# xXCoffeeColaXc/WeatherConverter

Measured on AMD Instinct MI355X. Metric: 256x256 images/sec (T=1000 DDPM sample), higher is better.
Workload: dtype fp32-class (f16x3: 2-piece fp16 split MFMA, fp32 accumulate); 1 GPU; DDPM reverse sampling, UNet config.yaml @ 256px, 16 images/GPU, T=1000, 126 timed steps from t=999; global_batch=16, image_size=256, parallelism=single GPU, devices=1, hip_graph=True, stream_groups=2, x_finite=True

## Files before the change

weatherconverter_amd/csrc/wc_wino.hip:

```cpp
#include <stdlib.h>

#include "wc_x6.hpp"

#ifndef WC_ABL
#define WC_ABL 0
#endif
#ifndef WC_WINO_SCALAR
#define WC_WINO_SCALAR 0
#endif

namespace {

using namespace wcx6;

constexpr int NT = 256;

WC_DEVICE void wino_lds16(__amdgpu_buffer_rsrc_t srd, void* dst, unsigned voff, int soff) {
    __builtin_amdgcn_raw_ptr_buffer_load_lds(srd, (__attribute__((address_space(3))) void*)dst, 16, voff, soff, 0, 0);
}

struct WDev {
    const float* src0;
    int C0, ldc0;
    const float* scale;
    const float* shift;
    const float* src1;
    int C1, ldc1;
    int B, H, W, N;
    const void* w;
    const float* bias;
    const float* temb;
    int temb_ld;
    const float* res;
    int ldres;
    float* out;
    int ldo;
    int nck0, nck1;
    int a_exp;
    const float* abound;
    const float* wsinv;
    float* absmax;
    float* gn_part;
    int gn_ncb, gn_sw, gn_c0, gn_np64;
    int tiles_x, tiles_y, ntiles_n;
    const unsigned char* vpre;
    long vimg;
    const float* gb_x;
    int gb_ldx, gb_silu;
    const float* gb_sc0;
    const float* gb_sh0;
    const float* gb_gamma;
    const float* gb_beta;
    float* gb_part;
    float* gb_part3;
};

WC_DEVICE float wino_silu_grad(float y) {
    const float s = 1.0f / (1.0f + __expf(-y));
    return s * (1.0f + y * (1.0f - s));
}

constexpr int VPL = WC_SINGLE16 ? 8 : 16;

template <int TH, int BN, int MB = 2, int NW = 4, bool VP = false>
struct WTile {
    static constexpr int NT = 64 * NW;
    static constexpr int WAVES_N = BN / 32;
    static constexpr int WAVES_M = NW / WAVES_N;
    static_assert(WAVES_N * WAVES_M == NW && WAVES_M * 4 * MB == TH, "each wave owns 4 MB rows x 8 tiles x 32 channels");
    static constexpr int PBN = BN > 128 ? 128 : BN;
    static constexpr int HR = TH + 2;
    static constexpr int PSTR = HR * 128 + (VP ? 0 : 16);
    static constexpr int DPIECES = VPL * HR * 8 / 64;
    static_assert(!VP || VPL * HR * 8 == DPIECES * 64, "VP: the halo stage is a whole number of 1-KiB pieces");
    static constexpr int DPW = (DPIECES + NW - 1) / NW;
    static constexpr int HSTAGE = 16 * PSTR;
    static constexpr int CPSTR = TH * 128 + 16;
    static constexpr int CSTAGE = 8 * CPSTR;
    static constexpr int ITEMS = HR * 16;
    static constexpr int I_PER_T = (ITEMS + NT - 1) / NT;
    static constexpr int C_PER_T = TH * 16 * 4 / NT;
    static constexpr int BSTEP = PBN * 64;
    static constexpr int STEPS = 12;
};

WC_DEVICE int wg_grp(int r) { return ((r >= 4 && r < 12) || (r >= 16 && r < 20) || r >= 28) ? 1 : 0; }
WC_DEVICE int wg_idx(int r) { return r < 4 ? r : r < 12 ? r - 4 : r < 20 ? r - 8 : r < 28 ? r - 12 : r - 16; }
WC_DEVICE int wg_row(int r) { return 2 * wg_grp(r) + (wg_idx(r) >> 3); }
WC_DEVICE int wg_tile(int r) { return wg_idx(r) & 7; }

template <int TH, int BN, int PRO, bool RES, int MB = 2, int NW = 4>
__global__ __launch_bounds__(64 * NW) __attribute__((amdgpu_waves_per_eu(MB == 4 ? 1 : 2, MB == 4 ? 1 : 2)))
void conv3x3_wino_kernel(WDev p) {
    static_assert((PRO == 2 || PRO == 0 || PRO == 3) && !(PRO == 0 && RES),
                  "GN+SiLU (+ residual), pre-split GN+SiLU (+ residual) or one raw segment");
    constexpr bool VP = PRO == 3;
    using T = WTile<TH, BN, MB, NW, VP>;
    constexpr int NT = T::NT;
    extern __shared__ __attribute__((aligned(16))) unsigned char smem[];
    unsigned char* const cbase = smem + 2 * T::HSTAGE;

    const int tid = threadIdx.x;
    const int lane = tid & 63;
    const int wave = tid >> 6;
    const int wm = wave / T::WAVES_N;
    const int wn = wave % T::WAVES_N;

    const int nblk = gridDim.x;
    int bid = blockIdx.x;
    {
        int q = nblk / 8, r = nblk % 8, xcd = bid % 8;
        bid = (xcd < r ? xcd * (q + 1) : r * (q + 1) + (xcd - r) * q) + bid / 8;
    }
    const int tile_n = bid % p.ntiles_n;
    int tt = bid / p.ntiles_n;
    const int txi = tt % p.tiles_x;
    tt /= p.tiles_x;
    const int tyi = tt % p.tiles_y;
    const int b = tt / p.tiles_y;
    const int y0 = tyi * TH, x0 = txi * 16, n0 = tile_n * BN;

    int s_exp = p.a_exp;
    if ((RES || PRO == 0) && p.abound) {
        const float bnd = p.abound[b];
        const int e = (int)((__float_as_uint(bnd) >> 23) & 0xffu) - 127;
        if (bnd > 0.f) s_exp = min(s_exp, (PRO == 0 ? 12 : 13) - e);
        s_exp = max(s_exp, -100);
    }
    const float ascale = ldexpf(1.0f, s_exp), ainv = ldexpf(1.0f, -s_exp);
    const int S0 = T::STEPS * p.nck0;
    const int S = S0 + (RES ? p.nck1 : 0);
    constexpr bool RI = RES && (T::C_PER_T <= 2 || MB == 4);
    const int nri = RI ? min(p.nck0, p.nck1) : 0;
    const int ntail = RES ? p.nck1 - nri : 0;
    constexpr int WPT = T::PBN / 32;
    const unsigned wtile = (unsigned)(tile_n * (BN / T::PBN) + wn / WPT) * (unsigned)(S * T::BSTEP);

    const __amdgpu_buffer_rsrc_t srd0 = make_srd(p.src0);
    const __amdgpu_buffer_rsrc_t srd1 = make_srd(RES ? p.src1 : p.src0);
    const __amdgpu_buffer_rsrc_t srdw = make_srd(p.w);
    const __amdgpu_buffer_rsrc_t srdsc = make_srd(PRO == 2 ? p.scale : p.src0);
    const __amdgpu_buffer_rsrc_t srdsh = make_srd(PRO == 2 ? p.shift : p.src0);
    const __amdgpu_buffer_rsrc_t srdv = make_srd(VP ? (const void*)(p.vpre + (long)b * p.vimg) : (const void*)p.src0);
    unsigned voff[VP ? T::DPW : 1];
    if constexpr (VP) {
#pragma unroll
        for (int i = 0; i < T::DPW; ++i) {
            const int f = (wave + NW * i) * 64 + lane;
            const int P = f / (T::HR * 8), r = (f >> 3) % T::HR, tl = f & 7;
            const int y = y0 - 1 + r;
            voff[i] = (unsigned)y < (unsigned)p.H ? (unsigned)(((P * p.H + y) * (p.W / 2) + (x0 >> 1) + tl) * 16) : OOB;
        }
    }
    const int vchunk = VPL * p.H * (p.W / 2) * 16;
    auto dma_halo = [&](int c, int hs) {
        if constexpr (VP) {
            unsigned char* dst = smem + hs * T::HSTAGE + wave * 1024;
#pragma unroll
            for (int i = 0; i < T::DPW; ++i)
                if (T::DPIECES % NW == 0 || wave + NW * i < T::DPIECES)
                    wino_lds16(srdv, dst + i * NW * 1024, voff[i], c * vchunk);
        }
    };

    const int q = tid & 3;
    int hbase[T::I_PER_T];
    unsigned hin[T::I_PER_T];
    int hwr[T::I_PER_T];
    const int hpx = p.ldc0 * 4;
#pragma unroll
    for (int j = 0; j < T::I_PER_T; ++j) {
        const int i = tid + NT * j;
        const int hrow = i >> 4, tp = (i >> 2) & 3;
        const bool valid = i < T::ITEMS;
        const int iy = y0 - 1 + hrow;
        hin[j] = 0;
#pragma unroll
        for (int k = 0; k < 6; ++k) {
            const int ix = x0 - 1 + 4 * tp + k;
            const bool inb = valid && (unsigned)iy < (unsigned)p.H && (unsigned)ix < (unsigned)p.W;
            hin[j] |= (inb ? 1u : 0u) << k;
        }
        hbase[j] = (((b * p.H + iy) * p.W + x0 - 1 + 4 * tp) * p.ldc0 + 4 * q) * 4;
        hwr[j] = valid ? (q >> 1) * T::PSTR + (hrow * 8 + 2 * tp) * 16 + (q & 1) * 8 : -1;
    }
    f32x4 rh[T::I_PER_T][6];
    f32x4 rsc, rsh;
    auto load_ss = [&](int c) {
        if constexpr (PRO == 2) {
            const unsigned o = (unsigned)(b * p.C0 + c * 16 + 4 * q) * 4u;
            rsc = bload_f4(srdsc, o);
            rsh = bload_f4(srdsh, o);
        }
    };
    auto load_slot = [&](int j, int c) {
#pragma unroll
        for (int k = 0; k < 6; ++k)
            rh[j][k] = bload_f4s(srd0, ((hin[j] >> k) & 1u) ? (unsigned)(hbase[j] + k * hpx) : OOB, c * 64);
    };
    auto load_halo = [&](int c) {
        if constexpr (VP) return;
#pragma unroll
        for (int j = 0; j < T::I_PER_T; ++j) load_slot(j, c);
        load_ss(c);
    };
#if WC_WINO_SCALAR
    const float cu = -1.4426950408889634f * ainv;
    auto prologue = [&](int j, int k0, int k1) {
        if constexpr (PRO == 2) {
            if (j == 0 && k0 == 0) {
                rsc = rsc * ascale;
                rsh = rsh * ascale;
            }
        }
        auto act = [&](f32x4 a) {
#pragma unroll
            for (int e = 0; e < 4; ++e) {
                float v;
                if constexpr (PRO == 2) {
                    const float ap = __builtin_fmaf(a[e], rsc[e], rsh[e]);
                    const float r = __builtin_amdgcn_rcpf(1.0f + __builtin_amdgcn_exp2f(ap * cu));
                    v = ap * r;
                } else {
                    v = a[e] * ascale;
                }
                a[e] = v;
            }
            return a;
        };
#pragma unroll
        for (int k = k0; k < k1; ++k) {
            const f32x4 zero = {0.f, 0.f, 0.f, 0.f};
#if WC_WINO_SCALAR == 2
            rh[j][k] = ((hin[j] >> k) & 1u) ? act(rh[j][k]) : zero;
#else
            const f32x4 a = act(rh[j][k]);
            rh[j][k] = ((hin[j] >> k) & 1u) ? a : zero;
#endif
        }
    };
#else
    auto prologue = [&](int j, int k0, int k1) {
#pragma unroll
        for (int k = k0; k < k1; ++k) {
            f32x4 a = rh[j][k];
            if constexpr (PRO == 2 && !(WC_ABL & 2)) {
                a = a * rsc + rsh;
                if constexpr (!(WC_ABL & 1)) {
                    a.x = silu_fast(a.x); a.y = silu_fast(a.y);
                    a.z = silu_fast(a.z); a.w = silu_fast(a.w);
                }
            }
            rh[j][k] = ((hin[j] >> k) & 1u) ? a * ascale : f32x4{0.f, 0.f, 0.f, 0.f};
        }
    };
#endif
    auto transform = [&](int j, int t, int hs, int p0 = 0, int p1 = 4) {
        if (hwr[j] < 0) return;
        unsigned char* base = smem + hs * T::HSTAGE + hwr[j] + t * 16;
        const f32x4 d0 = rh[j][2 * t], d1 = rh[j][2 * t + 1], d2 = rh[j][2 * t + 2], d3 = rh[j][2 * t + 3];
#if WC_WINO_SCALAR
        f32x4 V[4];
#pragma unroll
        for (int e = 0; e < 4; ++e) {
            V[0][e] = d0[e] - d2[e];
            V[1][e] = d1[e] + d2[e];
            V[2][e] = d2[e] - d1[e];
            V[3][e] = d1[e] - d3[e];
        }
#else
        const f32x4 V[4] = {d0 - d2, d1 + d2, d2 - d1, d1 - d3};
#endif
#pragma unroll
        for (int pos = p0; pos < p1; ++pos) {
            u32x2 a0, a1;
            split2_f16(V[pos], a0, a1);
            unsigned char* d = base + pos * 2 * T::PSTR;
            *reinterpret_cast<u32x2*>(d) = a0;
            *reinterpret_cast<u32x2*>(d + 8 * T::PSTR) = a1;
        }
    };
    auto write_items = [&](int hs) {
        if constexpr (VP) return;
#pragma unroll
        for (int j = 0; j < T::I_PER_T; ++j) {
            prologue(j, 0, 6);
            transform(j, 0, hs);
            transform(j, 1, hs);
        }
    };

    f32x4 rc[2][RES ? T::C_PER_T : 1];
    const int cpx = (tid >> 2) & 15, crow0 = tid >> 6;
    const unsigned coff0 = (unsigned)(((b * p.H + y0 + crow0) * p.W + x0 + cpx) * p.ldc1 + 4 * q);
    const unsigned cstep = (unsigned)(NW * p.W * p.ldc1);
    const int cwr0 = (cpx & 1) * 2 * T::CPSTR + (q >> 1) * T::CPSTR + (crow0 * 8 + (cpx >> 1)) * 16 + (q & 1) * 8;
    auto load_centre = [&](auto P, int c, bool live = true) {
        constexpr int PV = decltype(P)::value;
        const unsigned v = live ? coff0 * 4u : OOB;
#pragma unroll
        for (int j = 0; j < T::C_PER_T; ++j)
            rc[PV][j] = bload_f4s(srd1, v, (int)(((unsigned)j * cstep + (unsigned)c * 16u) * 4u));
    };
    auto write_centre = [&](auto P, int cs) {
        constexpr int PV = decltype(P)::value;
        unsigned char* base = cbase + cs * T::CSTAGE + cwr0;
        const float sg = (cpx & 1) ? -ascale : ascale;
#pragma unroll
        for (int j = 0; j < T::C_PER_T; ++j) {
            u32x2 a0, a1;
            split2_f16(rc[PV][j] * sg, a0, a1);
            unsigned char* d = base + j * NW * 8 * 16;
            *reinterpret_cast<u32x2*>(d) = a0;
            *reinterpret_cast<u32x2*>(d + 4 * T::CPSTR) = a1;
        }
    };

    const int l32 = lane & 31;
    const int half = lane >> 5;
    int abase[MB];
#pragma unroll
    for (int mb = 0; mb < MB; ++mb) abase[mb] = ((4 * MB * wm + 4 * mb + wg_row(l32)) * 8 + wg_tile(l32)) * 16;
    const unsigned wlane = (unsigned)(half * T::PBN * 16 + ((wn % WPT) * 32 + l32) * 16);

    u32x4 wreg[3][2];
    auto load_w = [&](int set, int st) {
        int s = st < S0 ? st : S0 + nri + (st - S0);
        s = s < S ? s : S - 1;
        const int off = (int)(wtile + (unsigned)s * T::BSTEP);
#pragma unroll
        for (int pc = 0; pc < 2; ++pc) wreg[set][pc] = bload_u4s(srdw, wlane + (unsigned)(pc * 2 * T::PBN * 16), off);
    };
    u32x4 wres[2];
    auto load_wres = [&](int r) {
        const int s = S0 + r < S ? S0 + r : S - 1;
        const int off = (int)(wtile + (unsigned)s * T::BSTEP);
#pragma unroll
        for (int pc = 0; pc < 2; ++pc) wres[pc] = bload_u4s(srdw, wlane + (unsigned)(pc * 2 * T::PBN * 16), off);
    };

    f32x16 acc[4][MB];
#pragma unroll
    for (int i = 0; i < 4; ++i)
#pragma unroll
        for (int j = 0; j < MB; ++j)
#pragma unroll
            for (int r = 0; r < 16; ++r) acc[i][j][r] = 0.f;

    u32x4 fa[2][MB][2];
    auto read_a = [&](int fs, int hs, int dy, int pos) {
        const unsigned char* ha = smem + hs * T::HSTAGE + (pos * 2 + half) * T::PSTR + dy * 128;
#pragma unroll
        for (int mb = 0; mb < MB; ++mb)
#pragma unroll
            for (int pc = 0; pc < 2; ++pc)
                fa[fs][mb][pc] = *reinterpret_cast<const u32x4*>(ha + pc * 8 * T::PSTR + abase[mb]);
    };
    auto mfma_a = [&](int fs, int set, int pos) {
#pragma unroll
        for (int mb = 0; mb < MB; ++mb) acc[pos][mb] = mfma_f16(fa[fs][mb][0], wreg[set][0], acc[pos][mb]);
#pragma unroll
        for (int mb = 0; mb < MB; ++mb) {
            acc[pos][mb] = mfma_f16c(fa[fs][mb][0], wreg[set][1], acc[pos][mb]);
            acc[pos][mb] = mfma_f16c(fa[fs][mb][1], wreg[set][0], acc[pos][mb]);
        }
    };
    auto compute_res = [&](const u32x4 (&w)[2], int cs) {
        const unsigned char* ca = cbase + cs * T::CSTAGE + half * T::CPSTR;
#pragma unroll
        for (int r = 0; r < 2; ++r) {
            u32x4 fr[MB][2];
#pragma unroll
            for (int mb = 0; mb < MB; ++mb)
#pragma unroll
                for (int pc = 0; pc < 2; ++pc)
                    fr[mb][pc] = *reinterpret_cast<const u32x4*>(ca + (pc * 4 + r * 2) * T::CPSTR + abase[mb]);
#pragma unroll
            for (int mb = 0; mb < MB; ++mb) {
                f32x16& a = acc[r ? 3 : 0][mb];
                a = mfma_f16(fr[mb][0], w[0], a);
                a = mfma_f16c(fr[mb][0], w[1], a);
                a = mfma_f16c(fr[mb][1], w[0], a);
            }
        }
    };

    const std::integral_constant<int, 0> I0;
    const std::integral_constant<int, 1> I1;
    const int pv0 = (p.nck0 - 1) & 1;
    load_halo(0);
    dma_halo(0, pv0);
    if constexpr (RI) load_centre(I0, 0, nri > 0);
    load_w(0, 0);
    load_w(1, 1);
    write_items(pv0);
    if constexpr (RI) write_centre(I0, pv0);
    if constexpr (VP) asm volatile("s_waitcnt vmcnt(0)" ::: "memory");
    __syncthreads();
    constexpr int HALO_AT = T::I_PER_T == 1 ? 2 : 3;
    auto load_at = [](int j) { return T::I_PER_T == 1 ? 2 : (j == 0 ? 3 : 7); };
    auto pro_at = [](int j) { return j == 0 ? 5 : 9; };
    auto slot_work = [&](int j, int k, int hs) {
        if constexpr (VP) return;
        if constexpr (WC_ABL & 4) {
            if (k >= 0 && k < 3) prologue(j, 2 * k, 2 * k + 2);
            return;
        }
        if constexpr (T::I_PER_T == 1) {
            if (k >= 0 && k < 3) prologue(j, 2 * k, 2 * k + 2);
            if (k >= 3 && k < 7) transform(j, (k - 3) >> 1, hs, ((k - 3) & 1) * 2, ((k - 3) & 1) * 2 + 2);
        } else {
            if (k == 0) prologue(j, 0, 6);
            if (k == 1 || k == 2) transform(j, k - 1, hs);
        }
    };
    auto chunk = [&](auto P, auto L, int c) {
        constexpr int PV = decltype(P)::value;
        constexpr bool LAST = decltype(L)::value != 0;
        read_a(0, PV, 0, 0);
#pragma unroll
        for (int st = 0; st < T::STEPS; ++st) {
            if (!(WC_ABL & 8) || c == 0) load_w((st + 2) % 3, T::STEPS * c + st + 2);
            if constexpr (!LAST) {
#pragma unroll
                for (int j = 0; j < T::I_PER_T; ++j)
                    if (!(WC_ABL & 32) && st == load_at(j)) load_slot(j, c + 1);
                if (st == HALO_AT) {
                    dma_halo(c + 1, PV ^ 1);
                    load_ss(c + 1);
                    if constexpr (RI) load_centre(I0, c + 1, c + 1 < nri);
                }
            } else if constexpr (RES) {
                if (st == HALO_AT) load_centre(I0, nri, ntail > 0);
                if (st == HALO_AT + 1) load_centre(I1, nri + 1, ntail > 1);
            }
            if constexpr (RI) {
                if (st == 9) load_wres(c);
            }
            __builtin_amdgcn_sched_barrier(0);
            if (st + 1 < T::STEPS && (!(WC_ABL & 64) || c == 0)) read_a((st + 1) & 1, PV, (st + 1) >> 2, (st + 1) & 3);
            mfma_a(st & 1, st % 3, st & 3);
            if constexpr (!LAST) {
#pragma unroll
                for (int j = 0; j < T::I_PER_T; ++j) slot_work(j, st - pro_at(j), PV ^ 1);
                if constexpr (RI) {
                    if (st == 9) write_centre(I0, PV ^ 1);
                }
            }
        }
        if constexpr (RES) {
            if constexpr (RI) {
                if (c < nri) compute_res(wres, PV);
            }
            if constexpr (LAST) {
                if (ntail > 0) write_centre(I0, 1);
            }
        }
        if constexpr (VP && !LAST) asm volatile("s_waitcnt vmcnt(4)" ::: "memory");
        if constexpr (!(WC_ABL & 16)) __syncthreads();
    };
    const std::integral_constant<int, 0> NL;
    const std::integral_constant<int, 1> LL;
    {
        int c = 0;
        if (pv0) chunk(I1, NL, c++);
        for (; c + 1 < p.nck0 - 1; c += 2) {
            chunk(I0, NL, c);
            chunk(I1, NL, c + 1);
        }
        chunk(I0, LL, p.nck0 - 1);
    }
    if constexpr (RES) {
        auto tstep = [&](auto P, int k) {
            constexpr int PV = decltype(P)::value;
            compute_res(wreg[PV], PV ^ 1);
            load_w(PV, S0 + k + 2);
            load_centre(P, nri + k + 2, k + 2 < ntail);
            __builtin_amdgcn_sched_barrier(0);
            if (k + 1 < ntail) write_centre(std::integral_constant<int, PV ^ 1>{}, PV);
            __syncthreads();
        };
        int k = 0;
        for (; k + 1 < ntail; k += 2) {
            tstep(I0, k);
            tstep(I1, k + 1);
        }
        if (k < ntail) tstep(I0, k);
    }

    const long img_px = (long)b * p.H * p.W;
    const __amdgpu_buffer_rsrc_t srd_out = make_srd(p.out + img_px * p.ldo);
    const __amdgpu_buffer_rsrc_t srd_res = make_srd(p.res ? p.res + img_px * p.ldres : p.out);
    const int n = n0 + wn * 32 + l32;
    const bool nok = n < p.N;
    float eadd = (nok && p.bias) ? p.bias[n] : 0.f;
    if (nok && p.temb) eadd += p.temb[b * p.temb_ld + n];
    const float emul = nok ? p.wsinv[n] * ainv : 0.f;
    float vmax = 0.f;
    float gs1 = 0.f, gs2 = 0.f, gs3 = 0.f;
    const int so_px = 4 * p.ldo;
    const int so_rs = 4 * p.ldres;
#pragma unroll
    for (int mb = 0; mb < MB; ++mb) {
        unsigned vo[4], vr[4];
#pragma unroll
        for (int j = 0; j < 4; ++j) {
            const int row = 8 * j + 4 * half;
            const int pix = (y0 + 4 * MB * wm + 4 * mb + wg_row(row)) * p.W + x0 + 2 * wg_tile(row);
            vo[j] = (unsigned)(pix * p.ldo + n) * 4u;
            vr[j] = (unsigned)(pix * p.ldres + (nok ? n : 0)) * 4u;
        }
        float rv[2][16];
        if (p.res) {
#pragma unroll
            for (int r = 0; r < 16; ++r) {
                rv[0][r] = bload_f1s(srd_res, vr[r >> 2], (r & 3) * 2 * so_rs);
                rv[1][r] = bload_f1s(srd_res, vr[r >> 2], ((r & 3) * 2 + 1) * so_rs);
            }
        }
#pragma unroll
        for (int r = 0; r < 16; ++r) {
            const float m0 = acc[0][mb][r], m1 = acc[1][mb][r], m2 = acc[2][mb][r], m3 = acc[3][mb][r];
            float ya = ((m0 + m1) + m2) * emul + eadd;
            float yb = ((m1 - m2) - m3) * emul + eadd;
            if (p.res) {
                ya += rv[0][r];
                yb += rv[1][r];
            }
            acc[0][mb][r] = ya;
            acc[1][mb][r] = yb;
            vmax = fmaxf(vmax, fmaxf(fabsf(ya), fabsf(yb)));
        }
        if constexpr (PRO == 0) {
            if (p.gb_part) {
                const __amdgpu_buffer_rsrc_t srd_x = make_srd(p.gb_x + img_px * p.gb_ldx);
                const int so_x = 4 * p.gb_ldx;
                float xv[2][16];
#pragma unroll
                for (int r = 0; r < 16; ++r) {
                    const int j = r >> 2;
                    const int row = 8 * j + 4 * half;
                    const int pix = (y0 + 4 * MB * wm + 4 * mb + wg_row(row)) * p.W + x0 + 2 * wg_tile(row);
                    const unsigned vx = nok ? (unsigned)(pix * p.gb_ldx + n) * 4u : OOB;
                    xv[0][r] = bload_f1s(srd_x, vx, (r & 3) * 2 * so_x);
                    xv[1][r] = bload_f1s(srd_x, vx, ((r & 3) * 2 + 1) * so_x);
                }
                const long bn = (long)b * p.N + (nok ? n : 0);
                const float sc0 = p.gb_sc0[bn], sh0 = p.gb_sh0[bn];
                const float ga = p.gb_gamma ? p.gb_gamma[nok ? n : 0] : 1.f;
                const float be = p.gb_beta ? p.gb_beta[nok ? n : 0] : 0.f;
#pragma unroll
                for (int r = 0; r < 16; ++r)
#pragma unroll
                    for (int e = 0; e < 2; ++e) {
                        const float xh = xv[e][r] * sc0 + sh0;
                        float d = acc[e][mb][r];
                        if (p.gb_silu) d *= wino_silu_grad(ga * xh + be);
                        gs1 += d;
                        gs2 += d * xh;
                        gs3 += xh;
                    }
            }
        }
        if (nok) {
            if constexpr (WC_ABL & 128) {
                float sum = 0.f;
#pragma unroll
                for (int r = 0; r < 16; ++r) sum += acc[0][mb][r] + acc[1][mb][r];
                if (sum == 1234.5678f) bstore_f1s(srd_out, vo[0], 0, sum);
            } else {
#pragma unroll
                for (int r = 0; r < 16; ++r) {
                    bstore_f1s(srd_out, vo[r >> 2], (r & 3) * 2 * so_px, acc[0][mb][r]);
                    bstore_f1s(srd_out, vo[r >> 2], ((r & 3) * 2 + 1) * so_px, acc[1][mb][r]);
                }
            }
        }
    }
    if (!nok) vmax = 0.f;
    if (p.absmax) block_absmax_atomic(p.absmax, b, vmax);
    if constexpr (PRO == 0) {
        if (p.gb_part) {
            gs1 += __shfl_xor(gs1, 32, 64);
            gs2 += __shfl_xor(gs2, 32, 64);
            gs3 += __shfl_xor(gs3, 32, 64);
            const int splits = p.tiles_y * p.tiles_x * T::WAVES_M;
            const long sp = (long)b * splits + ((long)tyi * p.tiles_x + txi) * T::WAVES_M + wm;
            if (nok && half == 0) {
                p.gb_part[(sp * p.N + n) * 2] = gs1;
                p.gb_part[(sp * p.N + n) * 2 + 1] = gs2;
                if (p.gb_part3) p.gb_part3[sp * p.N + n] = gs3;
            }
        }
    }
    if (p.gn_part) {
        const int r4 = tyi * (TH / 4) + MB * wm;
#pragma unroll
        for (int mb = 0; mb < MB; ++mb) {
            const f32x16 blk[2][1] = {{acc[0][mb]}, {acc[1][mb]}};
            GnTile g{p.gn_part, p.gn_ncb, p.gn_sw,
                     (long)b * p.gn_np64 + (long)(((r4 + mb) >> 1) * p.tiles_x + txi) * 2 + ((r4 + mb) & 1),
                     (p.gn_c0 + n0 + wn * 32) / 32};
            gn_tile_partials(blk, g, p.N - n0 - wn * 32 >= 32 ? 1 : 0);
        }
    }
}

template <int TH, int BN, int PRO, bool RES, int MB = 2, int NW = 4>
int launch_wino(const WDev& d, hipStream_t stream) {
    using T = WTile<TH, BN, MB, NW, PRO == 3>;
    constexpr int lds = 2 * T::HSTAGE + (RES ? 2 * T::CSTAGE : 0);
    static bool attr_set = false;
    if (!attr_set) {
        hipError_t e = hipFuncSetAttribute(reinterpret_cast<const void*>(&conv3x3_wino_kernel<TH, BN, PRO, RES, MB, NW>),
                                           hipFuncAttributeMaxDynamicSharedMemorySize, lds);
        if (e != hipSuccess) return (int)e;
        attr_set = true;
    }
    WDev p = d;
    p.tiles_x = p.W / 16;
    p.tiles_y = p.H / TH;
    p.ntiles_n = (p.N + BN - 1) / BN;
    dim3 grid(p.B * p.tiles_y * p.tiles_x * p.ntiles_n);
    WC_SET_NAME("conv3x3_wino_kernel", {WC_TI(TH), WC_TI(BN), WC_TI(PRO), WC_TB(RES), WC_TI(MB), WC_TI(NW)});
    hipLaunchKernelGGL((conv3x3_wino_kernel<TH, BN, PRO, RES, MB, NW>), grid, dim3(T::NT), lds, stream, p);
    WC_CHECK_LAUNCH();
    return WC_OK;
}

}

extern "C" int wc_conv3x3_wino_tile_n(int N) { return N <= 64 ? 64 : 128; }

namespace {

int wino_setup(const wc_conv_args* a, const void* w, int64_t w_bytes, int a_exp, const float* w_inv_scale,
               const float* a_bound, WDev& d, int& pro, bool& res, int& BN) {
    if (!a || !w || !a->out || !w_inv_scale) return WC_E_ARG;
    if (a->nseg < 1 || a->nseg > 2) return WC_E_ARG;
    const wc_conv_seg& s0 = a->seg[0];
    if (!s0.src || (s0.scale == nullptr) != (s0.shift == nullptr)) return WC_E_ARG;
    pro = s0.scale ? 2 : 0;
    if (pro == 2 && !s0.silu) return WC_E_ARG;
    if (pro == 0 && (!a_bound || a->nseg != 1)) return WC_E_ARG;
    if (a->act != WC_ACT_NONE) return WC_E_ARG;
    if (a_exp < -60 || a_exp > 60) return WC_E_ARG;
    BN = wc_conv3x3_wino_tile_n(a->N);
    const int TH = BN == 64 ? 16 : 8;
    if (s0.ntaps != 9 || s0.sy != 1 || s0.sx != 1 || s0.kbase != 0) return WC_E_SHAPE;
    for (int t = 0; t < 9; ++t)
        if (s0.dy[t] != t / 3 - 1 || s0.dx[t] != t % 3 - 1) return WC_E_SHAPE;
    if (s0.C <= 0 || s0.C % 16 || s0.ldc % 4 || (reinterpret_cast<uintptr_t>(s0.src) & 15)) return WC_E_SHAPE;
    if (a->B <= 0 || a->N <= 0 || s0.H != a->Hm || s0.W != a->Wm || a->Hm % TH || a->Wm % 16) return WC_E_SHAPE;
    if ((long)a->B * s0.H * s0.W * s0.ldc * 4 >= (1L << 31)) return WC_E_SHAPE;
    if (reinterpret_cast<uintptr_t>(w) & 15) return WC_E_SHAPE;
    d = WDev{};
    d.src0 = s0.src; d.C0 = s0.C; d.ldc0 = s0.ldc; d.scale = s0.scale; d.shift = s0.shift;
    d.nck0 = s0.C / 16;
    res = a->nseg == 2;
    if (res) {
        const wc_conv_seg& s1 = a->seg[1];
        if (!s1.src || s1.scale || !a_bound) return WC_E_ARG;
        if (s1.ntaps != 1 || s1.dy[0] != 0 || s1.dx[0] != 0 || s1.sy != 1 || s1.sx != 1) return WC_E_SHAPE;
        if (s1.H != s0.H || s1.W != s0.W || s1.kbase != 9 * s0.C) return WC_E_SHAPE;
        if (s1.C <= 0 || s1.C % 16 || s1.ldc % 4 || (reinterpret_cast<uintptr_t>(s1.src) & 15)) return WC_E_SHAPE;
        if ((long)a->B * s1.H * s1.W * s1.ldc * 4 >= (1L << 31)) return WC_E_SHAPE;
        d.src1 = s1.src; d.C1 = s1.C; d.ldc1 = s1.ldc; d.nck1 = s1.C / 16;
    }
    if (a->out_nchw || a->Ho != a->Hm || a->Wo != a->Wm || a->osy != 1 || a->osx != 1 || a->ooy || a->oox)
        return WC_E_SHAPE;
    if ((long)a->Hm * a->Wm * a->ldo * 4 >= (1L << 31) || (a->res && (long)a->Hm * a->Wm * a->ldres * 4 >= (1L << 31)))
        return WC_E_SHAPE;
    d.B = a->B; d.H = a->Hm; d.W = a->Wm; d.N = a->N;
    d.w = w; d.bias = a->bias; d.temb = a->temb; d.temb_ld = a->temb_ld;
    d.res = a->res; d.ldres = a->ldres; d.out = a->out; d.ldo = a->ldo;
    d.a_exp = a_exp - 1;
    d.abound = (res || pro == 0) ? a_bound : nullptr;
    d.wsinv = w_inv_scale;
    d.absmax = a->absmax_out;
    d.gn_part = a->gn_part;
    if (a->gn_part) {
        const int sw = a->gn_sw;
        if ((sw != 4 && sw != 8 && sw != 16 && sw != 32) || a->N % 32 || a->gn_c0 % 32 || a->gn_c0 < 0 ||
            a->gn_c0 + a->N > a->gn_ncb * 32 || a->gn_p64 != 0 || a->gn_np64 * 64 != a->Hm * a->Wm)
            return WC_E_SHAPE;
        d.gn_ncb = a->gn_ncb; d.gn_sw = sw; d.gn_c0 = a->gn_c0; d.gn_np64 = a->gn_np64;
    }
    const long ntn = (a->N + BN - 1) / BN;
    if (w_bytes != ntn * (12L * d.nck0 + d.nck1) * BN * 64 || w_bytes >= (1L << 31)) return WC_E_SHAPE;
    return WC_OK;
}

long wino_vimg(int C, int H, int W) { return (long)(C / 16) * VPL * H * (W / 2) * 16; }

#ifndef VS_IPT
#define VS_IPT 4
#endif
template <int NCK>
__global__ __launch_bounds__(256) void wino_vsplit_kernel(const float* __restrict__ src, int ldc, int B, int H,
                                                          int W, int C, const float* __restrict__ scale,
                                                          const float* __restrict__ shift, int a_exp1,
                                                          const float* __restrict__ res_bound,
                                                          unsigned char* __restrict__ vout, long vimg) {
    extern __shared__ __attribute__((aligned(16))) f32x4 act[];
    const int R = 256 / W, ngrp = C / (16 * NCK), nyb = (H + R - 1) / R;
    const int kg = blockIdx.x % ngrp;
    const int yb = (blockIdx.x / ngrp) % nyb;
    const int b = blockIdx.x / (ngrp * nyb);
    const int y0 = yb * R;
    const int tid = threadIdx.x;
    int s_exp = a_exp1;
    if (res_bound) {
        const float bnd = res_bound[b];
        const int e = (int)((__float_as_uint(bnd) >> 23) & 0xffu) - 127;
        if (bnd > 0.f) s_exp = min(s_exp, 13 - e);
        s_exp = max(s_exp, -100);
    }
    const float ascale = ldexpf(1.0f, s_exp);
    const int W2 = W + 2, items = R * W2 * 4 * NCK, cstride = R * W2 * 5;
    const int qt = tid % (4 * NCK), ct = kg * 16 * NCK + 4 * qt;
    const f32x4 sct = *reinterpret_cast<const f32x4*>(scale + (long)b * C + ct);
    const f32x4 sht = *reinterpret_cast<const f32x4*>(shift + (long)b * C + ct);
    for (int i0 = tid; i0 < items; i0 += VS_IPT * 256) {
        f32x4 v[VS_IPT];
        bool inb[VS_IPT];
        int slot[VS_IPT];
#pragma unroll
        for (int u = 0; u < VS_IPT; ++u) {
            const int i = min(i0 + u * 256, items - 1);
            const int px = (i / (4 * NCK)) % W2 - 1, r = (i / (4 * NCK)) / W2;
            const int y = y0 + r;
            inb[u] = (unsigned)px < (unsigned)W && y < H;
            v[u] = *reinterpret_cast<const f32x4*>(src + ((long)(b * H + min(y, H - 1)) * W + min(max(px, 0), W - 1)) * ldc + ct);
            slot[u] = (qt >> 2) * cstride + (r * W2 + px + 1) * 5 + (qt & 3);
        }
#pragma unroll
        for (int u = 0; u < VS_IPT; ++u) {
            if (i0 + u * 256 >= items) break;
            f32x4 a = v[u] * sct + sht;
            a.x = silu_fast(a.x); a.y = silu_fast(a.y);
            a.z = silu_fast(a.z); a.w = silu_fast(a.w);
            act[slot[u]] = inb[u] ? a * ascale : f32x4{0.f, 0.f, 0.f, 0.f};
        }
    }
    __syncthreads();
    const int T2 = W / 2;
    const int t = tid % T2, h = (tid / T2) & 1, r = tid / W;
    const int y = y0 + r;
    if (r >= R || y >= H) return;
    const long plane = (long)H * T2 * 16;
    const long frag = ((long)y * T2 + t) * 16;
#pragma unroll
    for (int ck = 0; ck < NCK; ++ck) {
        unsigned char* vb = vout + (long)b * vimg + (long)(kg * NCK + ck) * VPL * H * T2 * 16;
        u32x2 pc[2][4][2];
#pragma unroll
        for (int qq = 0; qq < 2; ++qq) {
            const f32x4* ar = act + ck * cstride + (r * W2 + 2 * t) * 5 + 2 * h + qq;
            const f32x4 d0 = ar[0], d1 = ar[5], d2 = ar[10], d3 = ar[15];
            const f32x4 V[4] = {d0 - d2, d1 + d2, d2 - d1, d1 - d3};
#pragma unroll
            for (int pos = 0; pos < 4; ++pos) split2_f16(V[pos], pc[qq][pos][0], pc[qq][pos][1]);
        }
#pragma unroll
        for (int pos = 0; pos < 4; ++pos)
#pragma unroll
            for (int piece = 0; piece < VPL / 8; ++piece)
                *reinterpret_cast<u32x4*>(vb + (piece * 8 + pos * 2 + h) * plane + frag) =
                    u32x4{pc[0][pos][piece].x, pc[0][pos][piece].y, pc[1][pos][piece].x, pc[1][pos][piece].y};
    }
}

}

extern "C" int wc_conv3x3_wino_f16x3(const wc_conv_args* a, const void* w, int64_t w_bytes, int a_exp,
                                     const float* w_inv_scale, const float* a_bound, void* stream) {
    WDev d;
    int pro, BN;
    bool res;
    const int st = wino_setup(a, w, w_bytes, a_exp, w_inv_scale, a_bound, d, pro, res, BN);
    if (st != WC_OK) return st;
    hipStream_t s = reinterpret_cast<hipStream_t>(stream);
    if (pro == 0) return BN == 64 ? launch_wino<16, 64, 0, false>(d, s) : launch_wino<8, 128, 0, false>(d, s);
    if (BN == 64) return res ? launch_wino<16, 64, 2, true>(d, s) : launch_wino<16, 64, 2, false>(d, s);
    return res ? launch_wino<8, 128, 2, true>(d, s) : launch_wino<8, 128, 2, false>(d, s);
}

extern "C" int wc_conv3x3_wino_gnb_splits(int N, int H, int W) {
    const int BN = wc_conv3x3_wino_tile_n(N), TH = BN == 64 ? 16 : 8;
    if (N <= 0 || H <= 0 || W <= 0 || H % TH || W % 16) return -1;
    const int waves_m = 4 / (BN / 32);
    return (H / TH) * (W / 16) * waves_m;
}

extern "C" int wc_conv3x3_wino_f16x3_gnb(const wc_conv_args* a, const void* w, int64_t w_bytes, int a_exp,
                                         const float* w_inv_scale, const float* a_bound, const wc_gnb_epi* g,
                                         void* stream) {
    WDev d;
    int pro, BN;
    bool res;
    const int st = wino_setup(a, w, w_bytes, a_exp, w_inv_scale, a_bound, d, pro, res, BN);
    if (st != WC_OK) return st;
    if (pro != 0 || !g || !g->x || !g->sc0 || !g->sh0 || !g->part) return WC_E_ARG;
    if (g->ldx < d.N || g->splits != wc_conv3x3_wino_gnb_splits(d.N, d.H, d.W)) return WC_E_SHAPE;
    if ((long)d.B * d.H * d.W * g->ldx * 4 >= (1L << 31)) return WC_E_SHAPE;
    d.gb_x = g->x; d.gb_ldx = g->ldx; d.gb_silu = g->silu ? 1 : 0;
    d.gb_sc0 = g->sc0; d.gb_sh0 = g->sh0; d.gb_gamma = g->gamma; d.gb_beta = g->beta;
    d.gb_part = g->part; d.gb_part3 = g->part3;
    hipStream_t s = reinterpret_cast<hipStream_t>(stream);
    return BN == 64 ? launch_wino<16, 64, 0, false>(d, s) : launch_wino<8, 128, 0, false>(d, s);
}

extern "C" int wc_wino_vsplit_bytes(int B, int C, int H, int W, int64_t* bytes) {
    if (!bytes || B <= 0 || C <= 0 || C % 16 || H <= 0 || W <= 0 || W % 16) return WC_E_SHAPE;
    *bytes = (int64_t)B * wino_vimg(C, H, W);
    return WC_OK;
}

extern "C" int wc_wino_vsplit_f16x3(const wc_conv_args* a, int a_exp, const float* a_bound, void* vout, int64_t v_bytes,
                                    void* stream) {
    if (!a || !vout || a->nseg < 1 || a->nseg > 2) return WC_E_ARG;
    const wc_conv_seg& s0 = a->seg[0];
    if (!s0.src || !s0.scale || !s0.shift || !s0.silu) return WC_E_ARG;
    if (a->nseg == 2 && !a_bound) return WC_E_ARG;
    if (a_exp < -60 || a_exp > 60) return WC_E_ARG;
    if (s0.C <= 0 || s0.C % 16 || s0.ldc % 4 || (reinterpret_cast<uintptr_t>(s0.src) & 15) || s0.W % 16)
        return WC_E_SHAPE;
    if ((reinterpret_cast<uintptr_t>(vout) & 15) || v_bytes != (int64_t)a->B * wino_vimg(s0.C, s0.H, s0.W))
        return WC_E_SHAPE;
    if (s0.W > 256) return WC_E_SHAPE;
    const int R = 256 / s0.W;
    const int nck = s0.C % 32 == 0 ? 2 : 1;
    const long nblk = (long)a->B * ((s0.H + R - 1) / R) * (s0.C / (16 * nck));
    const size_t lds = (size_t)nck * R * (s0.W + 2) * 5 * sizeof(f32x4);
    if (lds > 64 * 1024) return WC_E_SHAPE;
    hipStream_t st = reinterpret_cast<hipStream_t>(stream);
    const float* rb = a->nseg == 2 ? a_bound : nullptr;
    unsigned char* vo = reinterpret_cast<unsigned char*>(vout);
    const long vimg = wino_vimg(s0.C, s0.H, s0.W);
    if (nck == 2) {
        WC_SET_NAME("wino_vsplit_kernel", {WC_TI(2)});
        hipLaunchKernelGGL(wino_vsplit_kernel<2>, dim3((unsigned)nblk), dim3(256), lds, st, s0.src, s0.ldc, a->B, s0.H,
                           s0.W, s0.C, s0.scale, s0.shift, a_exp - 1, rb, vo, vimg);
    } else {
        WC_SET_NAME("wino_vsplit_kernel", {WC_TI(1)});
        hipLaunchKernelGGL(wino_vsplit_kernel<1>, dim3((unsigned)nblk), dim3(256), lds, st, s0.src, s0.ldc, a->B, s0.H,
                           s0.W, s0.C, s0.scale, s0.shift, a_exp - 1, rb, vo, vimg);
    }
    WC_CHECK_LAUNCH();
    return WC_OK;
}

extern "C" int wc_conv3x3_wino_f16x3_vp(const wc_conv_args* a, const void* w, int64_t w_bytes, int a_exp,
                                        const float* w_inv_scale, const float* a_bound, const void* vpre,
                                        int64_t v_bytes, void* stream) {
    WDev d;
    int pro, BN;
    bool res;
    const int st = wino_setup(a, w, w_bytes, a_exp, w_inv_scale, a_bound, d, pro, res, BN);
    if (st != WC_OK) return st;
    if (pro != 2 || !vpre || (reinterpret_cast<uintptr_t>(vpre) & 15)) return WC_E_ARG;
    d.vimg = wino_vimg(d.C0, d.H, d.W);
    if (v_bytes != (int64_t)d.B * d.vimg || d.vimg >= (1L << 31)) return WC_E_SHAPE;
    d.vpre = reinterpret_cast<const unsigned char*>(vpre);
    hipStream_t s = reinterpret_cast<hipStream_t>(stream);
    if (BN == 64) return res ? launch_wino<16, 64, 3, true>(d, s) : launch_wino<16, 64, 3, false>(d, s);
    return res ? launch_wino<8, 128, 3, true>(d, s) : launch_wino<8, 128, 3, false>(d, s);
}

extern "C" int wc_conv3x3_wino_f16x3_vp8(const wc_conv_args* a, const void* w, int64_t w_bytes, int a_exp,
                                         const float* w_inv_scale, const float* a_bound, const void* vpre,
                                         int64_t v_bytes, void* stream) {
    WDev d;
    int pro, BN;
    bool res;
    const int st = wino_setup(a, w, w_bytes, a_exp, w_inv_scale, a_bound, d, pro, res, BN);
    if (st != WC_OK) return st;
    if (pro != 2 || !vpre || (reinterpret_cast<uintptr_t>(vpre) & 15)) return WC_E_ARG;
    if (BN != 128 || d.N % 256) return WC_E_SHAPE;
    d.vimg = wino_vimg(d.C0, d.H, d.W);
    if (v_bytes != (int64_t)d.B * d.vimg || d.vimg >= (1L << 31)) return WC_E_SHAPE;
    d.vpre = reinterpret_cast<const unsigned char*>(vpre);
    hipStream_t s = reinterpret_cast<hipStream_t>(stream);
    return res ? launch_wino<8, 256, 3, true, 2, 8>(d, s) : launch_wino<8, 256, 3, false, 2, 8>(d, s);
}

namespace {

__device__ double wino_u(const float* row, int C0, int ky, int pos, int c) {
    const double g0 = row[(ky * 3 + 0) * C0 + c], g1 = row[(ky * 3 + 1) * C0 + c], g2 = row[(ky * 3 + 2) * C0 + c];
    switch (pos) {
        case 0: return g0;
        case 1: return ((g0 + g1) + g2) * 0.5;
        case 2: return ((g0 - g1) + g2) * 0.5;
        default: return g2;
    }
}

__device__ void wino_u8(const float* row, int ld, int ky, int pos, int c, double* v) {
    f32x4 g[3][2];
#pragma unroll
    for (int k = 0; k < 3; ++k) {
        g[k][0] = *reinterpret_cast<const f32x4*>(row + (ky * 3 + k) * ld + c);
        g[k][1] = *reinterpret_cast<const f32x4*>(row + (ky * 3 + k) * ld + c + 4);
    }
#pragma unroll
    for (int e = 0; e < 8; ++e) {
        const double g0 = g[0][e >> 2][e & 3], g1 = g[1][e >> 2][e & 3], g2 = g[2][e >> 2][e & 3];
        v[e] = pos == 0 ? g0 : pos == 1 ? ((g0 + g1) + g2) * 0.5 : pos == 2 ? ((g0 - g1) + g2) * 0.5 : g2;
    }
}

__device__ void pack_wino_row(const float* row3, int ld, bool vec, const float* rres, bool live, int n, int C0, int C1,
                              int BN, short* __restrict__ out, float* __restrict__ wsinv) {
    const int c8 = C0 / 8, n0 = 12 * c8, nall = n0 + C1 / 8;
    auto values = [&](int it, double* v) {
        if (it < n0) {
            const int kp = it / c8, c = (it - kp * c8) * 8;
            if (vec) {
                wino_u8(row3, ld, kp / 4, kp % 4, c, v);
            } else {
#pragma unroll
                for (int e = 0; e < 8; ++e) v[e] = wino_u(row3, ld, kp / 4, kp % 4, c + e);
            }
        } else {
            const int c = (it - n0) * 8;
#pragma unroll
            for (int e = 0; e < 8; ++e) v[e] = rres[c + e];
        }
    };
    double m = 0.0;
    if (live) {
        for (int it = threadIdx.x; it < nall; it += blockDim.x) {
            double v[8];
            values(it, v);
#pragma unroll
            for (int e = 0; e < 8; ++e) m = fmax(m, fabs(v[e]));
        }
    }
    __shared__ double red[256];
    red[threadIdx.x] = m;
    __syncthreads();
    for (int s = 128; s > 0; s >>= 1) {
        if ((int)threadIdx.x < s) red[threadIdx.x] = fmax(red[threadIdx.x], red[threadIdx.x + s]);
        __syncthreads();
    }
    const double amax = red[0];
    int sw = 0;
    if (amax > 0.0) {
        int e;
        const double mant = frexp(amax, &e);
        sw = (mant == 0.5 ? 15 : 14) - e;
        sw = sw < -60 ? -60 : sw > 60 ? 60 : sw;
    }
    const double scale = ldexp(1.0, sw);
    if (threadIdx.x == 0) wsinv[n] = ldexpf(1.0f, -sw);
    const int T = n / BN, nn = n % BN;
    const long rowlen = (long)(12 * (C0 / 16) + C1 / 16) * 2 * 2 * BN * 8;
    short* trow = out + (long)T * rowlen;
    const int plane = 2 * BN * 8;
    for (int it = threadIdx.x; it < nall; it += blockDim.x) {
        double v[8];
        if (live) values(it, v);
        else
#pragma unroll
            for (int e = 0; e < 8; ++e) v[e] = 0.0;
        long o;
        if (it < n0) {
            const int kp = it / c8, c = (it - kp * c8) * 8, ky = kp / 4, pos = kp % 4;
            const int chunk = c / 16, kh = (c % 16) / 8;
            o = ((((long)(chunk * 3 + ky) * 4 + pos) * 2 * 2 + kh) * BN + nn) * 8;
        } else {
            const int c = (it - n0) * 8;
            const int chunk = c / 16, kh = (c % 16) / 8;
            o = (long)(C0 / 16) * 12 * 2 * 2 * BN * 8 + (((long)chunk * 2 * 2 + kh) * BN + nn) * 8;
        }
        unsigned hp[4], lp[4];
#pragma unroll
        for (int e = 0; e < 8; e += 2) {
            unsigned short h0, l0, h1, l1;
            float a = (float)(v[e] * scale), b = (float)(v[e + 1] * scale);
            asm volatile("" : "+v"(a), "+v"(b));
            split2_one(a, h0, l0);
            split2_one(b, h1, l1);
            hp[e / 2] = (unsigned)h0 | ((unsigned)h1 << 16);
            lp[e / 2] = (unsigned)l0 | ((unsigned)l1 << 16);
        }
        *reinterpret_cast<u32x4*>(trow + o) = u32x4{hp[0], hp[1], hp[2], hp[3]};
        *reinterpret_cast<u32x4*>(trow + o + plane) = u32x4{lp[0], lp[1], lp[2], lp[3]};
    }
}

__global__ __launch_bounds__(256) void pack_wino_kernel(const float* __restrict__ w, int K, int N, int C0, int C1,
                                                        int BN, short* __restrict__ out, float* __restrict__ wsinv) {
    const int n = blockIdx.x;
    const bool live = n < N;
    const float* row = w + (long)(live ? n : 0) * K;
    pack_wino_row(row, C0, false, row + 9 * C0, live, n, C0, C1, BN, out, wsinv);
}

__device__ void stage_row3(const float* __restrict__ w, bool transposed, int N, int n, int C0, float* row3) {
    const int lim = 9 * C0, ld = C0 + 4;
    for (int i0 = threadIdx.x; i0 < lim; i0 += 8 * 256) {
        float v[8];
#pragma unroll
        for (int k = 0; k < 8; ++k) {
            const int i = i0 + k * 256;
            const int c = i / 9, t = i - 9 * c;
            v[k] = i < lim ? (transposed ? w[((long)c * N + n) * 9 + t] : w[(long)n * lim + i]) : 0.f;
        }
#pragma unroll
        for (int k = 0; k < 8; ++k) {
            const int i = i0 + k * 256;
            const int c = i / 9, t = i - 9 * c;
            if (i < lim) row3[(transposed ? 8 - t : t) * ld + c] = v[k];
        }
    }
}

template <bool TRANSPOSED>
__global__ __launch_bounds__(256) void pack_wino_raw_kernel(const float* __restrict__ w, const float* __restrict__ wres,
                                                            int N, int C0, int C1, int BN, short* __restrict__ out,
                                                            float* __restrict__ wsinv) {
    extern __shared__ float row3[];
    const int n = blockIdx.x;
    const bool live = n < N;
    if (live) stage_row3(w, TRANSPOSED, N, n, C0, row3);
    __syncthreads();
    pack_wino_row(row3, C0 + 4, true, wres + (long)(live ? n : 0) * C1, live, n, C0, C1, BN, out, wsinv);
}

__global__ __launch_bounds__(256) void pack_wino_batch_kernel(const wc_wino_pack_job* __restrict__ jobs, int njobs) {
    extern __shared__ float row3[];
    __shared__ int s_wg0[256];
    const int g = blockIdx.x;
    const bool lds = njobs <= 256;
    if (lds && (int)threadIdx.x < njobs) s_wg0[threadIdx.x] = jobs[threadIdx.x].wg0;
    __syncthreads();
    int lo = 0, hi = njobs - 1;
    while (lo < hi) {
        const int mid = (lo + hi + 1) >> 1;
        if ((lds ? s_wg0[mid] : jobs[mid].wg0) <= g) lo = mid;
        else hi = mid - 1;
    }
    const wc_wino_pack_job jb = jobs[lo];
    const int n = g - jb.wg0;
    const bool live = n < jb.N;
    const int C0 = jb.C0, N = jb.N;
    if (live) stage_row3(jb.w, jb.transposed != 0, N, n, C0, row3);
    __syncthreads();
    pack_wino_row(row3, C0 + 4, true, jb.wres + (long)(live ? n : 0) * jb.C1, live, n, C0, jb.C1, jb.BN,
                  reinterpret_cast<short*>(jb.out), jb.wsinv);
}

}

extern "C" int wc_pack_wino(const float* w, int N, int C0, int C1, void* out, int64_t out_bytes, float* w_inv_scale,
                            void* stream) {
    if (!w || !out || !w_inv_scale) return WC_E_ARG;
    if (N <= 0 || C0 <= 0 || C0 % 16 || C1 < 0 || C1 % 16) return WC_E_SHAPE;
    const int BN = wc_conv3x3_wino_tile_n(N);
    const long ntn = (N + BN - 1) / BN;
    if (out_bytes != ntn * (12L * (C0 / 16) + C1 / 16) * BN * 64) return WC_E_SHAPE;
    hipLaunchKernelGGL(pack_wino_kernel, dim3((unsigned)(ntn * BN)), dim3(256), 0, reinterpret_cast<hipStream_t>(stream),
                       w, 9 * C0 + C1, N, C0, C1, BN, reinterpret_cast<short*>(out), w_inv_scale);
    wc_last_kernel = "pack_wino_kernel";
    WC_CHECK_LAUNCH();
    return WC_OK;
}

extern "C" int wc_pack_wino_batch(const wc_wino_pack_job* jobs, int njobs, int total_wg, int max_c0, void* stream) {
    if (!jobs || njobs < 0 || total_wg < 0) return WC_E_ARG;
    if (njobs == 0) return WC_OK;
    if (max_c0 <= 0 || 9L * (max_c0 + 4) * 4 > 64 * 1024 || total_wg <= 0) return WC_E_SHAPE;
    hipLaunchKernelGGL(pack_wino_batch_kernel, dim3((unsigned)total_wg), dim3(256), (size_t)9 * (max_c0 + 4) * sizeof(float),
                       reinterpret_cast<hipStream_t>(stream), jobs, njobs);
    wc_last_kernel = "pack_wino_batch_kernel";
    WC_CHECK_LAUNCH();
    return WC_OK;
}

extern "C" int wc_pack_wino_raw(const float* w, const float* wres, int N, int C0, int C1, int transposed, void* out,
                                int64_t out_bytes, float* w_inv_scale, void* stream) {
    if (!w || !out || !w_inv_scale || (C1 && !wres) || (transposed && C1)) return WC_E_ARG;
    if (N <= 0 || C0 <= 0 || C0 % 16 || C1 < 0 || C1 % 16 || 9L * (C0 + 4) * 4 > 64 * 1024) return WC_E_SHAPE;
    const int BN = wc_conv3x3_wino_tile_n(N);
    const long ntn = (N + BN - 1) / BN;
    if (out_bytes != ntn * (12L * (C0 / 16) + C1 / 16) * BN * 64) return WC_E_SHAPE;
    const size_t lds = (size_t)9 * (C0 + 4) * sizeof(float);
    hipStream_t s = reinterpret_cast<hipStream_t>(stream);
    if (transposed)
        hipLaunchKernelGGL(pack_wino_raw_kernel<true>, dim3((unsigned)(ntn * BN)), dim3(256), lds, s, w, wres, N, C0, C1,
                           BN, reinterpret_cast<short*>(out), w_inv_scale);
    else
        hipLaunchKernelGGL(pack_wino_raw_kernel<false>, dim3((unsigned)(ntn * BN)), dim3(256), lds, s, w, wres, N, C0,
                           C1, BN, reinterpret_cast<short*>(out), w_inv_scale);
    wc_last_kernel = "pack_wino_raw_kernel";
    WC_CHECK_LAUNCH();
    return WC_OK;
}
```

Measured before the change: 0.6817 images/s.

## Deepen vp8 Winograd conv halo ring to four LDS buffers with half the barriers

Adds an NH template parameter so the pre-split 8-wave Winograd conv kernel can use a four-deep LDS ring for halo and centre stages, prefetching two chunks ahead and syncing only every other chunk. The goal is to hide global-to-LDS DMA latency and cut __syncthreads overhead in the main loop. It also makes the wave index scalar via readfirstlane. The cost is double the LDS footprint for this variant, which may lower occupancy, plus a more complex buffer-index scheme.

```diff
diff --git a/weatherconverter_amd/csrc/wc_wino.hip b/weatherconverter_amd/csrc/wc_wino.hip
--- a/weatherconverter_amd/csrc/wc_wino.hip
+++ b/weatherconverter_amd/csrc/wc_wino.hip
@@ -7,6 +7,9 @@
 #endif
 #ifndef WC_WINO_SCALAR
 #define WC_WINO_SCALAR 0
+#endif
+#ifndef WC_WINO_VP8_NH
+#define WC_WINO_VP8_NH 4
 #endif
 
 namespace {
@@ -62,8 +65,9 @@
 
 constexpr int VPL = WC_SINGLE16 ? 8 : 16;
 
-template <int TH, int BN, int MB = 2, int NW = 4, bool VP = false>
+template <int TH, int BN, int MB = 2, int NW = 4, bool VP = false, int NH = 2>
 struct WTile {
+    static_assert(NH == 2 || (NH == 4 && VP), "a ring of two buffers, or of four in a pre-split form");
     static constexpr int NT = 64 * NW;
     static constexpr int WAVES_N = BN / 32;
     static constexpr int WAVES_M = NW / WAVES_N;
@@ -82,6 +86,7 @@
     static constexpr int C_PER_T = TH * 16 * 4 / NT;
     static constexpr int BSTEP = PBN * 64;
     static constexpr int STEPS = 12;
+    static constexpr int lds(bool res) { return NH * HSTAGE + (res ? NH * CSTAGE : 0); }
 };
 
 WC_DEVICE int wg_grp(int r) { return ((r >= 4 && r < 12) || (r >= 16 && r < 20) || r >= 28) ? 1 : 0; }
@@ -89,20 +94,20 @@
 WC_DEVICE int wg_row(int r) { return 2 * wg_grp(r) + (wg_idx(r) >> 3); }
 WC_DEVICE int wg_tile(int r) { return wg_idx(r) & 7; }
 
-template <int TH, int BN, int PRO, bool RES, int MB = 2, int NW = 4>
+template <int TH, int BN, int PRO, bool RES, int MB = 2, int NW = 4, int NH = 2>
 __global__ __launch_bounds__(64 * NW) __attribute__((amdgpu_waves_per_eu(MB == 4 ? 1 : 2, MB == 4 ? 1 : 2)))
 void conv3x3_wino_kernel(WDev p) {
     static_assert((PRO == 2 || PRO == 0 || PRO == 3) && !(PRO == 0 && RES),
                   "GN+SiLU (+ residual), pre-split GN+SiLU (+ residual) or one raw segment");
     constexpr bool VP = PRO == 3;
-    using T = WTile<TH, BN, MB, NW, VP>;
+    using T = WTile<TH, BN, MB, NW, VP, NH>;
     constexpr int NT = T::NT;
     extern __shared__ __attribute__((aligned(16))) unsigned char smem[];
-    unsigned char* const cbase = smem + 2 * T::HSTAGE;
+    unsigned char* const cbase = smem + NH * T::HSTAGE;
 
     const int tid = threadIdx.x;
     const int lane = tid & 63;
-    const int wave = tid >> 6;
+    const int wave = NW == 8 ? __builtin_amdgcn_readfirstlane(tid >> 6) & (NW - 1) : tid >> 6;
     const int wm = wave / T::WAVES_N;
     const int wn = wave % T::WAVES_N;
 
@@ -153,13 +158,13 @@
         }
     }
     const int vchunk = VPL * p.H * (p.W / 2) * 16;
-    auto dma_halo = [&](int c, int hs) {
+    auto dma_halo = [&](int c, int hs, bool live = true) {
         if constexpr (VP) {
             unsigned char* dst = smem + hs * T::HSTAGE + wave * 1024;
 #pragma unroll
             for (int i = 0; i < T::DPW; ++i)
                 if (T::DPIECES % NW == 0 || wave + NW * i < T::DPIECES)
-                    wino_lds16(srdv, dst + i * NW * 1024, voff[i], c * vchunk);
+                    wino_lds16(srdv, dst + i * NW * 1024, live ? voff[i] : OOB, live ? c * vchunk : 0);
         }
     };
 
@@ -387,16 +392,21 @@
 
     const std::integral_constant<int, 0> I0;
     const std::integral_constant<int, 1> I1;
-    const int pv0 = (p.nck0 - 1) & 1;
+    const int pv0 = (p.nck0 - 1) & (NH - 1);
+    const int pv1 = (pv0 - 1) & (NH - 1);
     load_halo(0);
     dma_halo(0, pv0);
+    if constexpr (NH == 4) dma_halo(1, pv1, p.nck0 > 1);
     if constexpr (RI) load_centre(I0, 0, nri > 0);
+    if constexpr (RI && NH == 4) load_centre(I1, 1, nri > 1);
     load_w(0, 0);
     load_w(1, 1);
     write_items(pv0);
     if constexpr (RI) write_centre(I0, pv0);
+    if constexpr (RI && NH == 4) write_centre(I1, pv1);
     if constexpr (VP) asm volatile("s_waitcnt vmcnt(0)" ::: "memory");
     __syncthreads();
+    if constexpr (NH == 4) read_a(0, pv0, 0, 0);
     constexpr int HALO_AT = T::I_PER_T == 1 ? 2 : 3;
     auto load_at = [](int j) { return T::I_PER_T == 1 ? 2 : (j == 0 ? 3 : 7); };
     auto pro_at = [](int j) { return j == 0 ? 5 : 9; };
@@ -417,7 +427,11 @@
     auto chunk = [&](auto P, auto L, int c) {
         constexpr int PV = decltype(P)::value;
         constexpr bool LAST = decltype(L)::value != 0;
-        read_a(0, PV, 0, 0);
+        constexpr int AH = NH / 2;
+        constexpr int FB = (PV + AH) & (NH - 1);
+        constexpr int NX = (PV + NH - 1) & (NH - 1);
+        constexpr bool BAR = NH == 2 || LAST || !(PV & 1);
+        if constexpr (NH == 2) read_a(0, PV, 0, 0);
 #pragma unroll
         for (int st = 0; st < T::STEPS; ++st) {
             if (!(WC_ABL & 8) || c == 0) load_w((st + 2) % 3, T::STEPS * c + st + 2);
@@ -426,9 +440,10 @@
                 for (int j = 0; j < T::I_PER_T; ++j)
                     if (!(WC_ABL & 32) && st == load_at(j)) load_slot(j, c + 1);
                 if (st == HALO_AT) {
-                    dma_halo(c + 1, PV ^ 1);
+                    if constexpr (NH == 2) dma_halo(c + 1, FB);
+                    else dma_halo(c + AH, FB, c + AH < p.nck0);
                     load_ss(c + 1);
-                    if constexpr (RI) load_centre(I0, c + 1, c + 1 < nri);
+                    if constexpr (RI) load_centre(I0, c + AH, c + AH < nri);
                 }
             } else if constexpr (RES) {
                 if (st == HALO_AT) load_centre(I0, nri, ntail > 0);
@@ -439,12 +454,15 @@
             }
             __builtin_amdgcn_sched_barrier(0);
             if (st + 1 < T::STEPS && (!(WC_ABL & 64) || c == 0)) read_a((st + 1) & 1, PV, (st + 1) >> 2, (st + 1) & 3);
+            if constexpr (!BAR) {
+                if (st + 1 == T::STEPS) read_a(0, NX, 0, 0);
+            }
             mfma_a(st & 1, st % 3, st & 3);
             if constexpr (!LAST) {
 #pragma unroll
-                for (int j = 0; j < T::I_PER_T; ++j) slot_work(j, st - pro_at(j), PV ^ 1);
+                for (int j = 0; j < T::I_PER_T; ++j) slot_work(j, st - pro_at(j), FB);
                 if constexpr (RI) {
-                    if (st == 9) write_centre(I0, PV ^ 1);
+                    if (st == 9) write_centre(I0, FB);
                 }
             }
         }
@@ -453,15 +471,19 @@
                 if (c < nri) compute_res(wres, PV);
             }
             if constexpr (LAST) {
-                if (ntail > 0) write_centre(I0, 1);
-            }
-        }
-        if constexpr (VP && !LAST) asm volatile("s_waitcnt vmcnt(4)" ::: "memory");
-        if constexpr (!(WC_ABL & 16)) __syncthreads();
+                if (ntail > 0) write_centre(I0, NH == 2 ? 1 : 2);
+            }
+        }
+        constexpr bool ABL_HERE = !(WC_ABL & 512) || (VP && NW == 8);
+        if constexpr (BAR) {
+            if constexpr (VP && !LAST && !((WC_ABL & 256) && ABL_HERE)) asm volatile("s_waitcnt vmcnt(4)" ::: "memory");
+            if constexpr (!((WC_ABL & 16) && ABL_HERE)) __syncthreads();
+            if constexpr (NH == 4 && !LAST) read_a(0, NX, 0, 0);
+        }
     };
     const std::integral_constant<int, 0> NL;
     const std::integral_constant<int, 1> LL;
-    {
+    if constexpr (NH == 2) {
         int c = 0;
         if (pv0) chunk(I1, NL, c++);
         for (; c + 1 < p.nck0 - 1; c += 2) {
@@ -469,15 +491,30 @@
             chunk(I1, NL, c + 1);
         }
         chunk(I0, LL, p.nck0 - 1);
+    } else {
+        const std::integral_constant<int, 2> I2;
+        const std::integral_constant<int, 3> I3;
+        int c = 0;
+        if (pv0 == 3) chunk(I3, NL, c++);
+        if (pv0 >= 2) chunk(I2, NL, c++);
+        if (pv0 >= 1) chunk(I1, NL, c++);
+        for (; c < p.nck0 - 1; c += 4) {
+            chunk(I0, NL, c);
+            chunk(I3, NL, c + 1);
+            chunk(I2, NL, c + 2);
+            chunk(I1, NL, c + 3);
+        }
+        chunk(I0, LL, p.nck0 - 1);
     }
     if constexpr (RES) {
         auto tstep = [&](auto P, int k) {
             constexpr int PV = decltype(P)::value;
-            compute_res(wreg[PV], PV ^ 1);
+            constexpr int TB = NH == 2 ? PV ^ 1 : 2 + PV;
+            compute_res(wreg[PV], TB);
             load_w(PV, S0 + k + 2);
             load_centre(P, nri + k + 2, k + 2 < ntail);
             __builtin_amdgcn_sched_barrier(0);
-            if (k + 1 < ntail) write_centre(std::integral_constant<int, PV ^ 1>{}, PV);
+            if (k + 1 < ntail) write_centre(std::integral_constant<int, PV ^ 1>{}, TB ^ 1);
             __syncthreads();
         };
         int k = 0;
@@ -606,13 +643,14 @@
     }
 }
 
-template <int TH, int BN, int PRO, bool RES, int MB = 2, int NW = 4>
+template <int TH, int BN, int PRO, bool RES, int MB = 2, int NW = 4, int NH = 2>
 int launch_wino(const WDev& d, hipStream_t stream) {
-    using T = WTile<TH, BN, MB, NW, PRO == 3>;
-    constexpr int lds = 2 * T::HSTAGE + (RES ? 2 * T::CSTAGE : 0);
+    using T = WTile<TH, BN, MB, NW, PRO == 3, NH>;
+    constexpr int lds = T::lds(RES);
+    static_assert(lds <= 160 * 1024, "the CU's LDS");
     static bool attr_set = false;
     if (!attr_set) {
-        hipError_t e = hipFuncSetAttribute(reinterpret_cast<const void*>(&conv3x3_wino_kernel<TH, BN, PRO, RES, MB, NW>),
+        hipError_t e = hipFuncSetAttribute(reinterpret_cast<const void*>(&conv3x3_wino_kernel<TH, BN, PRO, RES, MB, NW, NH>),
                                            hipFuncAttributeMaxDynamicSharedMemorySize, lds);
         if (e != hipSuccess) return (int)e;
         attr_set = true;
@@ -622,8 +660,8 @@
     p.tiles_y = p.H / TH;
     p.ntiles_n = (p.N + BN - 1) / BN;
     dim3 grid(p.B * p.tiles_y * p.tiles_x * p.ntiles_n);
-    WC_SET_NAME("conv3x3_wino_kernel", {WC_TI(TH), WC_TI(BN), WC_TI(PRO), WC_TB(RES), WC_TI(MB), WC_TI(NW)});
-    hipLaunchKernelGGL((conv3x3_wino_kernel<TH, BN, PRO, RES, MB, NW>), grid, dim3(T::NT), lds, stream, p);
+    WC_SET_NAME("conv3x3_wino_kernel", {WC_TI(TH), WC_TI(BN), WC_TI(PRO), WC_TB(RES), WC_TI(MB), WC_TI(NW), WC_TI(NH)});
+    hipLaunchKernelGGL((conv3x3_wino_kernel<TH, BN, PRO, RES, MB, NW, NH>), grid, dim3(T::NT), lds, stream, p);
     WC_CHECK_LAUNCH();
     return WC_OK;
 }
@@ -882,7 +920,8 @@
     if (v_bytes != (int64_t)d.B * d.vimg || d.vimg >= (1L << 31)) return WC_E_SHAPE;
     d.vpre = reinterpret_cast<const unsigned char*>(vpre);
     hipStream_t s = reinterpret_cast<hipStream_t>(stream);
-    return res ? launch_wino<8, 256, 3, true, 2, 8>(d, s) : launch_wino<8, 256, 3, false, 2, 8>(d, s);
+    return res ? launch_wino<8, 256, 3, true, 2, 8, WC_WINO_VP8_NH>(d, s)
+               : launch_wino<8, 256, 3, false, 2, 8, WC_WINO_VP8_NH>(d, s);
 }
 
 namespace {
```

Result: faster. 0.6897 images/s, median of 6 (+1.2%).
